# HydrogenSulfate/LFT

Measured on AMD Instinct MI355X. Metric: LF patches/sec (5x5 angRes, 32x32 LR, 4xSR), higher is better.
Workload: dtype bf16; 1 GPU; LFT 5x5 angRes 4xSR inference, batch=4 per GPU, 32x32 LR patches; global_batch=4, parallelism=dp1 (independent shards), streams_per_gpu=1, hip_graph=True, steps_in_flight=2

## Files before the change

lft_amd/csrc/lft_api.hip:

```cpp
#include "../../include/lft_hip.h"
#include "../../include/lft_hip_test.h"
#include <hip/hip_runtime.h>
#include <stdint.h>

#include <cstdarg>
#include <cstdio>
#include <cmath>
#include <map>
#include <mutex>
#include <set>
#include <string>
#include <algorithm>
#include <type_traits>
#include <utility>
#include <vector>

#ifndef LFT_TU
#define LFT_TU 0
#endif

namespace {
#include "lft_kernels_a.cuh"
#include "lft_kernels_b.cuh"
#include "lft_metrics.cuh"
// ... 89 lines not shown

template <auto... Vs, typename V, typename F> int dispatch(V v, F&& f) {
    int rc = 0;
    if (((v == Vs && ((rc = f(std::integral_constant<decltype(Vs), Vs>{})), true)) || ...)) return rc;
    return fail(LFT_ERR_ARG, "internal: no kernel variant for %d", (int)v);
}
template <int V> using int_c = std::integral_constant<int, V>;
template <typename F> int by_prec(int prec, F&& f) {
    if (prec == LFT_PREC_F32) return f(float{});
    if (prec == LFT_PREC_BF16) return f(bf16_t{});
    return f(f16_t{});
}
inline size_t align256(size_t x) { return (x + 255) & ~(size_t)255; }

struct Dims {
    int B, A, V, h, w, hw, s, gp, gt, nchunk;
    long long ntok;
};

int make_dims(int B, int A, int h, int w, int s, int prec, Dims* d) {
    if (prec != LFT_PREC_F32 && prec != LFT_PREC_BF16 && prec != LFT_PREC_F16)
        return fail(LFT_ERR_ARG, "prec must be LFT_PREC_F32, LFT_PREC_BF16 or LFT_PREC_F16, got %d", prec);
    if (B < 1 || A < 1 || h < 1 || w < 1) return fail(LFT_ERR_SHAPE, "B, A, h, w must be positive (B=%d A=%d h=%d w=%d)", B, A, h, w);
    if (s != 2 && s != 4) return fail(LFT_ERR_SHAPE, "scale factor must be 2 or 4, got %d", s);
    if (A * A > 128) return fail(LFT_ERR_UNSUPPORTED, "angRes %d (A*A=%d views > 128) is not implemented in this build", A, A * A);
    if ((long long)B * A * A * h * w > (1LL << 27)) return fail(LFT_ERR_SHAPE, "too many tokens");
    d->B = B; d->A = A; d->V = A * A; d->h = h; d->w = w; d->hw = h * w; d->s = s;
    d->gp = (s + 2) * (s + 2); d->gt = (d->gp + 31) / 32; d->nchunk = 2 * s * s;
    d->ntok = (long long)B * d->V * d->hw;
    return 0;
}

constexpr int kFragsConv = 72, kFragsAng = 64, kFragsSpa1 = 240, kFragsSpa1NoQ = 208, kFragsSpa2 = 176;
inline int frags_up(const Dims& d) { return d.nchunk * (4 + 2 * d.gt); }

struct PackedLayout {
    size_t conv0_w, ln_ang[kLayers], ln_spa[kLayers], ang_pe, petok[kLayers], spa_pe_img;
    size_t w01, s_w01;
    size_t s_conv[3], s_ang[kLayers], s_spa1[kLayers], s_spa2[kLayers], s_up, total;
};

PackedLayout packed_layout(const Dims& d, int prec) {
    const size_t esz = prec == LFT_PREC_F32 ? 4 : 2, fragb = 64 * 8 * esz;
    PackedLayout L;
    size_t o = 0;
    auto take = [&](size_t bytes) { size_t r = o; o = align256(o + bytes); return r; };
    L.conv0_w = take(576 * 4);
    for (int l = 0; l < kLayers; ++l) { L.ln_ang[l] = take(256 * 4); L.ln_spa[l] = take(512 * 4); }
    L.ang_pe = take((size_t)((d.V + 31) / 32) * 2048 * 4);
    for (int l = 0; l < kLayers; ++l) L.petok[l] = take((size_t)((d.hw + 32 * kNwSpa1 - 1) / (32 * kNwSpa1)) * kNwSpa1 * 4096 * esz);
    L.spa_pe_img = take((size_t)d.hw * 64 * esz);
    const bool lp = prec != LFT_PREC_F32;
    L.w01 = take(lp ? 64 * kW01K * 4 : 0);
    L.s_conv[0] = take(kFragsConv * fragb);
    L.s_w01 = take(lp ? kW01Frags * fragb : 0);
    for (int i = 1; i < 3; ++i) L.s_conv[i] = take(kFragsConv * fragb);
    for (int l = 0; l < kLayers; ++l) {
        L.s_ang[l] = take(kFragsAng * fragb);
        L.s_spa1[l] = take(kFragsSpa1 * fragb);
        L.s_spa2[l] = take(kFragsSpa2 * fragb);
    }
    L.s_up = take((size_t)frags_up(d) * fragb);
    L.total = o;
    return L;
}

struct WorkLayout {
    size_t x0, feat, xa, xb, tok, q, k, v, o, g, status, total;
};
WorkLayout work_layout(const Dims& d, int prec) {
    const size_t esz = prec == LFT_PREC_F32 ? 4 : 2;
    WorkLayout W;
    size_t o = 0;
    auto take = [&](size_t bytes) { size_t r = o; o = align256(o + bytes); return r; };
    const size_t n = (size_t)d.ntok;
    W.x0 = take(n * 64 * esz); W.feat = take(n * 64 * esz); W.xa = take(n * 64 * esz); W.xb = take(n * 64 * esz);
    W.tok = take(n * 128 * esz); W.q = take(n * 128 * esz); W.k = take(n * 128 * esz); W.v = take(n * 128 * esz);
    W.o = take(n * 128 * esz);
    W.g = take(n * d.gp * 4);
    W.status = take(256);
    W.total = o;
    return W;
}

template <typename T> size_t lds_conv64(int w) { return WRing<T, kConv64Chunk, kNwConv>::LDS_BYTES + ConvIn<T, kNwConv>::bytes(w) + kNwConv * TileIO<2, T>::BYTES + kConvZeroRow; }
template <typename T> size_t lds_conv64_lr(int w) { return lds_conv64<T>(w) + std::max<size_t>(LrStage<kNwConv>::bytes(w), kConv0WBytes); }
constexpr size_t kLdsParams = 1024;
template <typename T, int CH = kSpaChunk> size_t lds_spa1(int w) {
    return WRing<T, CH, kNwSpa1>::LDS_BYTES + std::max<size_t>(ConvIn<T, kNwSpa1>::bytes(w), (size_t)kNwSpa1 * TileIO<4, T>::BYTES) + kLdsParams + kConvZeroRow;
}
template <typename T> size_t lds_spa2() { return WRing<T, kSpaChunk, kNwSpa2>::LDS_BYTES + kLdsParams + kNwSpa2 * TileIO<4, T>::BYTES; }
template <typename T> size_t lds_up() { return WRing<T, kUpChunk, kNwUp>::LDS_BYTES + kNwUp * TileIO<2, T>::BYTES; }
template <typename T> size_t lds_ang() { return (size_t)kFragsAng * 1024 * FragInfo<T>::PIECES + kLdsParams + 4 * TileIO<2, T>::BYTES; }
constexpr size_t kMaxLds = 160 * 1024;
template <typename K> int allow_lds(K kernel, size_t bytes, const char* name) {
// ... 59 lines not shown
    return dispatch<8, 16>(use8 ? 8 : 16, [&](auto CH) {
        return dispatch<true, false>(lm, [&](auto LM) {
            constexpr bool WQ = !(LM && sizeof(T) == 2);
            const size_t lds = CH == 8 ? l8 : l16;
            if (int rc = allow_lds(k_spa1<T, PE_ONLY, CH, LM, WQ>, lds, "k_spa1")) return rc;
            k_spa1<T, PE_ONLY, CH, LM, WQ><<<nwg, 64 * kNwSpa1, lds, st>>>(in, ws, ln, petok, tok, q, k, v, pe_out, nimg, d.h, d.w, status);
            return 0;
        });
    });
}

template <typename T>
int pack_impl(const float* const* P, void* packed, const Dims& d, int prec, hipStream_t st) {
    const PackedLayout L = packed_layout(d, prec);
    const float kAngScale = 0.35355339059327373f * LFT_LOG2E;
    const float kSpaScale = 0.25f * LFT_LOG2E;
    int rc;
    k_copy_f32<<<3, 256, 0, st>>>(P[0], at<float>(packed, L.conv0_w), 576);
    LFT_LAUNCH_OK("k_copy_f32");
    for (int i = 0; i < 3; ++i) {
        std::vector<PackOp> ops;
        conv_ops(ops, P[1 + i], 64);
        if ((rc = run_pack<T>(ops, at<T>(packed, L.s_conv[i]), kFragsConv, st))) return rc;
    }
    if constexpr (sizeof(T) == 2) {
        k_compose_w01<<<blocks_for(64 * kW01K, 256), 256, 0, st>>>(P[0], P[1], at<float>(packed, L.w01));
        LFT_LAUNCH_OK("k_compose_w01");
        std::vector<PackOp> ops{lin_op(at<float>(packed, L.w01), 0, 64, kW01K, 0, kW01K / 16, 0, 1.0f)};
        if ((rc = run_pack<ConvLrOp>(ops, at<ConvLrOp>(packed, L.s_w01), kW01Frags, st))) return rc;
    }
    k_pe_tables<T><<<blocks_for(std::max<long long>((long long)((d.V + 31) / 32) * 2048, (long long)d.hw * 64), 256), 256, 0, st>>>(
        at<float>(packed, L.ang_pe), at<T>(packed, L.spa_pe_img), d.V, d.h, d.w);
    LFT_LAUNCH_OK("k_pe_tables");
    for (int l = 0; l < kLayers; ++l) {
        const float* const* q = P + 4 + 18 * l;
        float* lnS = at<float>(packed, L.ln_spa[l]);
        float* lnA = at<float>(packed, L.ln_ang[l]);
        const int srcS[4] = {1, 2, 5, 6}, srcA[4] = {10, 11, 14, 15};
        for (int j = 0; j < 4; ++j) {
            k_copy_f32<<<1, 256, 0, st>>>(q[srcS[j]], lnS + 128 * j, 128);
            k_copy_f32<<<1, 256, 0, st>>>(q[srcA[j]], lnA + 64 * j, 64);
        }
        LFT_LAUNCH_OK("k_copy_f32");
        {
            std::vector<PackOp> ops;
            ops.push_back(lin_op(q[12], 0, 64, 64, 0, 4, 1, kAngScale));
            ops.push_back(lin_op(q[12], 64, 64, 64, 0, 4, 1, 1.0f));
            ops.push_back(lin_op(q[12], 128, 64, 64, 0, 4, 1, 1.0f));
            ops.push_back(lin_op(q[13], 0, 64, 64, 0, 4, 1, 1.0f));
            ops.push_back(lin_op(q[16], 0, 128, 64, 0, 4, 1, 1.0f));
            ops.push_back(lin_op(q[17], 0, 64, 128, 0, 8, 1, 1.0f));
            if ((rc = run_pack<T>(ops, at<T>(packed, L.s_ang[l]), kFragsAng, st))) return rc;
        }
        {
            std::vector<PackOp> ops;
            conv_ops(ops, q[0], 128);
            ops.push_back(lin_op(q[3], 256, 128, 128, 0, 8, 1, 1.0f));
            ops.push_back(lin_op(q[3], 128, 128, 128, 0, 8, 1, 1.0f));
            ops.push_back(lin_op(q[3], 0, 128, 128, 0, 8, 1, kSpaScale));
            if ((rc = run_pack<T>(ops, at<T>(packed, L.s_spa1[l]), kFragsSpa1, st))) return rc;
        }
        {
            std::vector<PackOp> ops;
            ops.push_back(lin_op(q[4], 0, 128, 128, 0, 8, (sizeof(T) == 2 && tok_lane_major<T>(d)) ? 1 : 0, 1.0f));
            for (int c = 0; c < 4; ++c) {
                ops.push_back(lin_op(q[7], 64 * c, 64, 128, 0, 8, 1, 1.0f));
                ops.push_back(lin_op(q[8], 0, 128, 256, 64 * c, 4, 1, 1.0f));
            }
            ops.push_back(lin_op(q[9], 0, 64, 128, 0, 8, 1, 1.0f));
            if ((rc = run_pack<T>(ops, at<T>(packed, L.s_spa2[l]), kFragsSpa2, st))) return rc;
        }
        if ((rc = launch_spa1<T, true>((unsigned)((d.hw + 32 * kNwSpa1 - 1) / (32 * kNwSpa1)), at<T>(packed, L.spa_pe_img), at<T>(packed, L.s_spa1[l]), nullptr, nullptr,
                                       nullptr, nullptr, nullptr, nullptr, at<T>(packed, L.petok[l]), 1, d, st, nullptr))) return rc;
        LFT_LAUNCH_OK("k_spa1<pe>");
    }
    {
        std::vector<PackOp> ops;
        for (int c = 0; c < d.nchunk; ++c) {
            ops.push_back(lin_op(P[76], 32 * c, 32, 64, 0, 4, 1, 1.0f));
            PackOp m = lin_op(P[77], 0, d.gp, 0, 32 * c, 2, 1, 1.0f);
            m.kind = 1; m.s = d.s; m.ntiles = d.gt;
            ops.push_back(m);
        }
        if ((rc = run_pack<T>(ops, at<T>(packed, L.s_up), frags_up(d), st))) return rc;
    }
    return 0;
}

void launch_assemble(const float* lr, const float* g, float* out, int B, int A, int h, int w, int s, hipStream_t st, int gld = 0, unsigned* status = nullptr) {
    const dim3 tg((unsigned)((A * w + 7) / 8) * (unsigned)((A * h + 7) / 8) * (unsigned)B);
    if (!gld) gld = (s + 2) * (s + 2);
    if (s == 2) k_assemble_t<2><<<tg, 256, 0, st>>>(lr, g, out, B, A, h, w, gld, status);
    else k_assemble_t<4><<<tg, 256, 0, st>>>(lr, g, out, B, A, h, w, gld, status);
}

template <typename T>
int init_features_x0(const void* packed, const PackedLayout& L, const float* lr, T* x0, T* ta, T* tb, T* feat, const Dims& d, hipStream_t st) {
    const int nimg = d.B * d.V, nwg = nimg * ((d.hw + 32 * kNwConv - 1) / (32 * kNwConv));
    const size_t lds = lds_conv64<T>(d.w);
    int rc;
    if ((rc = allow_lds(k_conv64<T, 0>, lds, "k_conv64"))) return rc;
    if ((rc = allow_lds(k_conv64<T, 1>, lds, "k_conv64"))) return rc;
    k_conv0<T><<<dim3((unsigned)((d.hw + kConv0Tok - 1) / kConv0Tok), (unsigned)nimg), 256, 0, st>>>(lr, at<float>(packed, L.conv0_w), x0, d.B, d.A, d.h, d.w);
// ... 59 lines not shown
}
template <typename T>
int spa_part_a(const void* packed, const PackedLayout& L, int l, const T* in, void* ws, const WorkLayout& W, const Dims& d, hipStream_t st) {
    const int nimg = d.B * d.V, nwg = nimg * ((d.hw + 32 * kNwSpa1 - 1) / (32 * kNwSpa1));
    int rc;
    if ((rc = launch_spa1<T, false>((unsigned)nwg, in, at<T>(packed, L.s_spa1[l]), at<float>(packed, L.ln_spa[l]), at<T>(packed, L.petok[l]),
                                    at<T>(ws, W.tok), at<T>(ws, W.q), at<T>(ws, W.k), at<T>(ws, W.v), nullptr, nimg, d, st, at<unsigned>(ws, W.status)))) return rc;
    LFT_LAUNCH_OK("k_spa1");
    return 0;
}
template <typename F> int with_tail_variant(bool skip, bool tok_lm, bool out_lm, F&& launch) {
    if (out_lm) {
        if (!(skip && tok_lm)) return fail(LFT_ERR_ARG, "internal: lane-major output needs the skip variant and lane-major tokens");
        return launch(std::true_type{}, std::true_type{}, std::true_type{});
    }
    return dispatch<true, false>(skip, [&](auto SK) {
        return dispatch<true, false>(tok_lm, [&](auto LM) { return launch(SK, LM, std::false_type{}); });
    });
}
template <typename T>
int spa_part_b(const void* packed, const PackedLayout& L, int l, const T* skip, T* out, void* ws, const WorkLayout& W,
               const Dims& d, hipStream_t st, bool out_lm = false) {
    const int nimg = d.B * d.V;
    T *tok = at<T>(ws, W.tok), *q = at<T>(ws, W.q), *k = at<T>(ws, W.k), *v = at<T>(ws, W.v), *o = at<T>(ws, W.o);
    const float* ln = at<float>(packed, L.ln_spa[l]);
    const bool lm = tok_lane_major<T>(d);
    int rc;
    if constexpr (sizeof(T) == 2) {
        const unsigned ntile = (unsigned)(nimg * ((d.h + kAttTY - 1) / kAttTY) * ((d.w + kAttTX - 1) / kAttTX));
        if ((rc = with_tail_variant(skip, lm, out_lm, [&](auto SK, auto LM, auto YL) {
                 if (int r = allow_lds(k_spa_b<T, SK, LM, YL>, kSpaBLds, "k_spa_b")) return r;
                 k_spa_b<T, SK, LM, YL><<<ntile, 256, kSpaBLds, st>>>(tok, q, k, v, at<T>(packed, L.s_spa2[l]), ln, skip, out, d.h, d.w,
                                                                      at<unsigned>(ws, W.status), at<T>(packed, L.s_spa1[l]) + (size_t)kFragsSpa1NoQ * 512,
                                                                      at<T>(packed, L.petok[l]));
                 return 0;
             }))) return rc;
        LFT_LAUNCH_OK("k_spa_b");
        return 0;
    } else {
        const unsigned tiles = (unsigned)(((d.w + kWaTX - 1) / kWaTX) * ((d.h + kWaTY - 1) / kWaTY) * nimg);
        if ((rc = allow_lds(k_win_attn_lds<0, true>, kWaLds, "k_win_attn_lds"))) return rc;
        k_win_attn_lds<0, true><<<dim3(tiles, 4), 256, kWaLds, st>>>(reinterpret_cast<const float*>(q), reinterpret_cast<const float*>(k),
                                                                     reinterpret_cast<const float*>(v), reinterpret_cast<float*>(o),
                                                                     nullptr, nullptr, nullptr, nullptr, nullptr, d.h, d.w, 128);
        LFT_LAUNCH_OK("k_spa_attn");
        const unsigned nb = blocks_for(d.ntok, 32 * kNwSpa2);
        if ((rc = with_tail_variant(skip, lm, out_lm, [&](auto SK, auto LM, auto YL) {
                 if (int r = allow_lds(k_spa2<T, SK, LM, YL>, lds_spa2<T>(), "k_spa2")) return r;
                 k_spa2<T, SK, LM, YL><<<nb, 64 * kNwSpa2, lds_spa2<T>(), st>>>(tok, o, at<T>(packed, L.s_spa2[l]), ln, skip, out, d.ntok, at<unsigned>(ws, W.status));
                 return 0;
             }))) return rc;
        LFT_LAUNCH_OK("k_spa2");
        return 0;
    }
}
template <typename T>
int spa_block(const void* packed, const PackedLayout& L, int l, const T* in, const T* skip, T* out, void* ws, const WorkLayout& W,
              const Dims& d, hipStream_t st, bool out_lm = false) {
    int rc;
    if ((rc = spa_part_a<T>(packed, L, l, in, ws, W, d, st))) return rc;
    return spa_part_b<T>(packed, L, l, skip, out, ws, W, d, st, out_lm);
}
template <typename T>
int upsample(const void* packed, const PackedLayout& L, const T* body, const float* lr, float* out, void* ws, const WorkLayout& W,
             const Dims& d, hipStream_t st, bool in_lm = false) {
    float* g = at<float>(ws, W.g);
    const unsigned nb = blocks_for(d.ntok, 32 * kNwUp);
// ... 893 lines not shown
```

lft_amd/csrc/lft_kernels_a.cuh:

```cuda
#pragma once
#include "lft_common.cuh"

struct PackOp {
    const float* src;
    int kind, row0, nrows, ntiles, ld, kmul, kadd, k0, ksteps, kmap, frag0, s;
    float scale;
    int order;
};
__host__ __device__ __forceinline__ int wfrag_index(int OT, int KS, int ot, int ks) {
    const int g = ot >> 2, G = OT - 4 * g < 4 ? OT - 4 * g : 4;
    return 4 * g * KS + ks * G + (ot & 3);
}
__host__ __device__ __forceinline__ void wfrag_coords(int OT, int KS, int lf, int order, int& nt, int& ks) {
    if (!order) { nt = lf / KS; ks = lf % KS; return; }
    const int gl = (OT - 1) >> 2, g = lf / (4 * KS) < gl ? lf / (4 * KS) : gl, G = OT - 4 * g < 4 ? OT - 4 * g : 4, rem = lf - 4 * g * KS;
    ks = rem / G; nt = 4 * g + rem % G;
}
constexpr int LFT_PACK_MAXOPS = 40;
struct PackArgs {
    int nops;
    PackOp op[LFT_PACK_MAXOPS];
};

LFT_DEV float upm_entry(const float* __restrict__ w3, int n, int kk, int s) {
// ... 169 lines not shown
        const char* row = inb ? lds_in + slot * CI::ROW_BYTES : zero_row;
        const int sw = inb ? CI::swz(slot) : 0;
#pragma unroll
        for (int ks = 0; ks < 4; ++ks) {
            Frag<T> b;
            if constexpr (sizeof(T) == 2) {
                b.v = __builtin_bit_cast(typename H16<T>::v8, load_raw16(row + (((2 * ks + hh) ^ sw) * 16)));
            } else {
                b.lo = __builtin_bit_cast(f32x4, load_raw16(row + (((4 * ks + 2 * hh) ^ sw) * 16)));
                b.hi = __builtin_bit_cast(f32x4, load_raw16(row + (((4 * ks + 2 * hh + 1) ^ sw) * 16)));
            }
#pragma unroll
            for (int nt = 0; nt < NT; ++nt) mma(ring.next(), b, acc[nt]);
        }
    }
}

constexpr int kNwConv = 4;
constexpr int kConv64Chunk = 12;

typedef f16_t ConvLrOp;
constexpr int kW01K = 96, kW01Frags = 12;
__host__ __device__ __forceinline__ int conv01_row_channel(int rho) { return (rho & ~12) | ((rho & 4) << 1) | ((rho & 8) >> 1); }
__global__ void k_compose_w01(const float* __restrict__ w0, const float* __restrict__ w1, float* __restrict__ w01) {
    const int idx = blockIdx.x * blockDim.x + threadIdx.x;
    if (idx >= 64 * kW01K) return;
    const int rho = idx / kW01K, k = idx - rho * kW01K;
    float v = 0.0f;
    if (k < 81) {
        const int o = conv01_row_channel(rho), t1 = k / 9, t0 = k - 9 * t1;
        for (int c = 0; c < 64; ++c) v += w1[o * 576 + c * 9 + t1] * w0[c * 9 + t0];
    }
    w01[idx] = v;
}
LFT_DEV const float* lr_view(const float* __restrict__ lr, int im, int A, int h, int w) {
    const int V = A * A, b = im / V, v = im - b * V, a1 = v / A, a2 = v - a1 * A;
    return lr + (size_t)b * (A * h) * (A * w) + (size_t)(a1 * h) * (A * w) + a2 * w;
}
template <int NW> struct LrStage {
    static __host__ __device__ int width(int w) { return w + 4; }
    static __host__ __device__ int max_rows(int w) { return (32 * NW + 2 * w + 1) / w + 6; }
    static __host__ __device__ int bytes(int w) { return (max_rows(w) * width(w) * 4 + 15) & ~15; }
};
constexpr int kConv0WBytes = 9 * 64 * 4;
LFT_DEV void conv0_w_stage(const float* __restrict__ w0, float* wl) {
    float wv[3];
#pragma unroll
    for (int k = 0; k < 3; ++k) wv[k] = w0[min((int)threadIdx.x + 256 * k, 575)];
#pragma unroll
    for (int k = 0; k < 3; ++k) {
        const int i = (int)threadIdx.x + 256 * k, ch = i / 9, t = i - ch * 9;
        if (i < 576) wl[t * 64 + ch] = wv[k];
    }
}
LFT_DEV void conv0_taps_load(const float* __restrict__ img, int ldi, int y, int x, int h, int w, float (&val)[9]) {
#pragma unroll
    for (int t = 0; t < 9; ++t) {
        const int yy = y + t / 3 - 1, xx = x + t % 3 - 1;
        val[t] = img[min(max(yy, 0), h - 1) * ldi + min(max(xx, 0), w - 1)];
    }
}
template <typename T>
LFT_DEV void conv0_token_acc(const float (&tap)[9], const float* wl, int y, int x, int h, int w, int hh, f32x16 (&rr)[2]) {
    float val[9];
#pragma unroll
    for (int t = 0; t < 9; ++t) {
// ... 462 lines not shown
```

lft_amd/csrc/lft_kernels_b.cuh:

```cuda
#pragma once
#include "lft_common.cuh"
#include "lft_kernels_a.cuh"

constexpr int kUpChunk = 8;
constexpr int kSpaChunk = 16;
constexpr int kSpaOcc = 2;
constexpr int kNwSpa1 = 4, kNwSpa2 = 4, kNwUp = 8;
template <typename T, bool PE_ONLY, int CH = kSpaChunk, bool TOKLM = false, bool WITH_Q = true, int NW = kNwSpa1>
__global__ __launch_bounds__(64 * NW, kSpaOcc) void k_spa1(const T* __restrict__ X, const T* __restrict__ ws,
                                              const float* __restrict__ ln, const T* __restrict__ petok,
                                              T* __restrict__ TOK, T* __restrict__ Q, T* __restrict__ K, T* __restrict__ Vv,
                                              T* __restrict__ pe_out, int nimg, int h, int w, unsigned* __restrict__ status) {
    extern __shared__ __attribute__((aligned(16))) char smem[];
    const int lane = threadIdx.x & 63, r = lane & 31, hh = lane >> 5, wave = threadIdx.x >> 6;
    constexpr int TT = 32 * NW;
    const int hw = h * w, tpi = (hw + TT - 1) / TT;
    const int bid = xcd_tile(blockIdx.x, gridDim.x);
    const int im = bid / tpi, p0 = (bid % tpi) * TT;
    const int tl = wave * 32 + r, p = p0 + tl;
    const bool ok = p < hw;
    LFT_STAMP(0);
    typename RawPiece<T>::type pe_raw[16];
    if (!PE_ONLY) load_lane_major_raw<4, T>(petok + (size_t)((p0 >> 5) + wave) * 4096, lane, pe_raw);
    char* lds_in = smem + WRing<T, CH, NW>::LDS_BYTES;
// ... 101 lines not shown
    LFT_STAMP(18);
#pragma unroll
    for (int nt = 0; nt < 4; ++nt) n[nt] = t[nt];
    unsigned bad = 0;
    layernorm_acc<4>(n, lds_ln, lds_ln + 128, hh, bad);
    acc_frags<4, T>(n, f);
    LFT_STAMP(19);
#pragma unroll
    for (int c = 0; c < 4; ++c) {
        f32x16 hid[2];
        zero_acc<2>(hid);
        linear_ring<2, 8, T>(ring, f, hid);
        Frag<T> hf[4];
        acc_frags_relu<2>(hid, hf);
        linear_ring<4, 4, T>(ring, hf, t);
    }
    LFT_STAMP(20);
    acc_frags<4, T>(t, f);
    f32x16 y[2];
    zero_acc<2>(y);
    linear_ring<2, 8, T>(ring, f, y);
    if (SKIP) {
#pragma unroll
        for (int nt = 0; nt < 2; ++nt) y[nt] += sk[nt];
    }
    LFT_STAMP(21);
    if constexpr (YLM) store_tile_lm<2, T>(Y + tb * 64, lane, y);
    else store_tile<2, T>(Y + tb * 64, nvalid, lane, y, scr);
    LFT_STAMP(22);
    publish_status(status, bad);
}

constexpr int kSpaBChunk = 8;
constexpr int kAdTile = kAttHR * kAttHC * 64;
constexpr int kAdPerWave = 2 * kAdTile / 1024 / 4;
static_assert(2 * kAdTile == 4 * kAdPerWave * 1024, "the K and V tiles must split into whole pieces over 4 waves");
constexpr int kSpaBLds = 4 * kAdTile + 2048;
constexpr int kSpaBSlotsA = (2 * kAdTile) / (kSpaBChunk * 1024);
constexpr int kSpaBSlotsB = 2;
constexpr int kSpaBSlots = kSpaBSlotsA + kSpaBSlotsB;
constexpr int kSpaBScratchOfs = 16384;
static_assert(kSpaBScratchOfs + 4 * TileIO<4, bf16_t>::BYTES <= 2 * kAdTile, "scratch must fit buffer B");
static_assert(kSpaBSlotsB * kSpaBChunk * 1024 <= kSpaBScratchOfs, "the ring slots in buffer B must end before the scratch");

template <typename T> LFT_DEV void q_load_async(const T* p0, const T* p1, raw16& a, raw16& b) {
    asm volatile("global_load_dwordx4 %0, %2, off\n\tglobal_load_dwordx4 %1, %3, off" : "=&v"(a), "=&v"(b) : "v"(p0), "v"(p1) : "memory");
}
LFT_DEV void ld16_async(const void* p, raw16& d) { asm volatile("global_load_dwordx4 %0, %1, off" : "=v"(d) : "v"(p) : "memory"); }
template <int OFS> LFT_DEV void ld16_async_ofs(const void* p, raw16& d) {
    static_assert(OFS >= 0 && OFS < 4096, "global_load immediate offset");
    asm volatile("global_load_dwordx4 %0, %1, off offset:%2" : "=v"(d) : "v"(p), "n"(OFS) : "memory");
}
LFT_DEV void ld16_async_x8(const char* p, raw16 (&d)[8]) {
    const char* p2 = p + 4096;
    ld16_async_ofs<0>(p, d[0]); ld16_async_ofs<1024>(p, d[1]); ld16_async_ofs<2048>(p, d[2]); ld16_async_ofs<3072>(p, d[3]);
    ld16_async_ofs<0>(p2, d[4]); ld16_async_ofs<1024>(p2, d[5]); ld16_async_ofs<2048>(p2, d[6]); ld16_async_ofs<3072>(p2, d[7]);
}
template <int N> LFT_DEV void wait_vm_8(raw16 (&r)[8]) {
    asm volatile("s_waitcnt vmcnt(%8)" : "+v"(r[0]), "+v"(r[1]), "+v"(r[2]), "+v"(r[3]), "+v"(r[4]), "+v"(r[5]), "+v"(r[6]), "+v"(r[7]) : "n"(N) : "memory");
    __builtin_amdgcn_sched_barrier(0);
}
template <int N> LFT_DEV void wait_vm_only() {
    asm volatile("s_waitcnt vmcnt(%0)" :: "n"(N) : "memory");
    __builtin_amdgcn_sched_barrier(0);
}
template <int N> LFT_DEV void wait_vm_q(raw16& a, raw16& b) {
    asm volatile("s_waitcnt vmcnt(%2)" : "+v"(a), "+v"(b) : "n"(N) : "memory");
    __builtin_amdgcn_sched_barrier(0);
}

template <typename T> LFT_DEV void q_head_pair(const raw16 (&wr)[8], const Frag<T> (&nf)[8], Frag<T>& q0, Frag<T>& q1) {
    f32x16 q;
#pragma unroll
    for (int i = 0; i < 16; ++i) q[i] = 0.0f;
#pragma unroll
    for (int ks = 0; ks < 8; ++ks) {
        Frag<T> wf;
        wf.v = __builtin_bit_cast(typename H16<T>::v8, wr[ks]);
        mma(wf, nf[ks], q);
    }
    q0 = acc_to_frag(q, 0, T());
    q1 = acc_to_frag(q, 1, T());
}

template <typename T, bool SKIP, bool TOKLM = false, bool YLM = false>
__global__ __launch_bounds__(256, 2) void k_spa_b(const T* __restrict__ TOK, const T* __restrict__ Q, const T* __restrict__ K,
                                                  const T* __restrict__ Vv, const T* __restrict__ ws, const float* __restrict__ ln,
                                                  const T* __restrict__ skip, T* __restrict__ Y, int h, int w, unsigned* __restrict__ status,
                                                  const T* __restrict__ wq, const T* __restrict__ petok) {
    static_assert(sizeof(T) == 2, "k_spa_b is the 16-bit (bf16 / f16) part B; fp32 uses k_win_attn_lds + k_spa2");
    typedef typename H16<T>::v8 V8;
    using Ring = WRingPipe<T, kSpaBChunk, 4, kSpaBSlots, 176>;
    extern __shared__ __attribute__((aligned(16))) char smem[];
    char* const bufA = smem;
    char* const bufB = smem + 2 * kAdTile;
    float* lds_ln = reinterpret_cast<float*>(smem + 4 * kAdTile);
    const int tiles_x = (w + kAttTX - 1) / kAttTX, tiles_y = (h + kAttTY - 1) / kAttTY;
    const int bid = xcd_tile(blockIdx.x, gridDim.x);
    const int tx = bid % tiles_x, ty = (bid / tiles_x) % tiles_y, im = bid / (tiles_x * tiles_y);
    const int lane = threadIdx.x & 63, r = lane & 31, hh = lane >> 5;
    const int wave = __builtin_amdgcn_readfirstlane(threadIdx.x >> 6);
    const int y0 = ty * kAttTY, x0 = tx * kAttTX, bxl = 8 * wave;
    const long long img0 = (long long)im * h * w;
    LFT_STAMP(16);
    const int qpx = 4 * (r >> 4) + (r & 3), qpy = (r >> 2) & 3;
    const int qy = y0 + qpy, qx = x0 + bxl + qpx;
    const long long qtok = img0 + min(qy, h - 1) * w + min(qx, w - 1);
    const T* qptr = TOKLM ? Q + (img0 + (long long)min(qy, h - 1) * w + x0) * 128 + (32 * hh + bxl + qpx) * 8
                               : Q + qtok * 128 + 8 * hh;
    constexpr int kQHead = TOKLM ? 512 : 16, kQPair = 2 * kQHead;
    int dofs[kAdPerWave];
    {
        const int s0 = (wave & 1) * kAdPerWave * 16 + (lane >> 2), piece = lane & 3;
        int row = s0 / kAttHC, col = s0 % kAttHC;
#pragma unroll
        for (int i = 0; i < kAdPerWave; ++i) {
            const int gy = min(max(y0 - 2 + row, 0), h - 1), gx = min(max(x0 - 2 + col, 0), w - 1);
            const int tk = gy * w + gx;
            const int pq = piece ^ att_swz(row, col);
            const int pconst = TOKLM ? ((pq >> 1) * 512 + (pq & 1) * 256) * 2 : pq * 16;
            dofs[i] = (TOKLM ? ((tk & ~31) << 8) + ((tk & 31) << 4) : tk * 256) + pconst;
            col += 16;
            if (col >= kAttHC) { col -= kAttHC; row += 1; }
        }
    }
    constexpr int kDmaPair = TOKLM ? 2048 : 64;
    const char* const dsrc = reinterpret_cast<const char*>((wave < 2 ? K : Vv) + img0 * 128);
    const int ddst = (wave < 2 ? 0 : kAdTile) + (wave & 1) * kAdPerWave * 1024;
    auto stage = [&](int hg, char* buf) {
        LFT_DMA_NOTE("DMA", kNoteKV, hg & 1);
#pragma unroll
        for (int i = 0; i < kAdPerWave; ++i) glds16_asm(dsrc + dofs[i] + hg * kDmaPair, buf + ddst + i * 1024);
    };
    const int g4 = lane >> 4, qi = lane & 15;
    f32x4 bias[2][4];
    int kb[2], vb[2];
    auto setup_tiles = [&]() __attribute__((always_inline)) {
    {
        const int wy0 = max(0, qy - 2), wy1 = min(h, qy + 3), cy0 = y0 - 2;
        const int ya = min(max(wy0 - cy0, 0), 8), yb = min(max(wy1 - cy0, 0), 8);
        const unsigned ymask = ((1u << yb) - 1u) & ~((1u << ya) - 1u);
        const int gy = g4 >> 1, gx4 = 4 * (g4 & 1);
#pragma unroll
        for (int b = 0; b < 2; ++b) {
            const int bqx = x0 + bxl + 4 * b + (lane & 3), cx0 = x0 + bxl + 4 * b - 2;
            const int wx0 = max(0, bqx - 2), wx1 = min(min(h, bqx + 3), w);
            const int xa = min(max(wx0 - cx0, 0), 8), xb = min(max(wx1 - cx0, 0), 8);
            const unsigned xs = (((1u << xb) - 1u) & ~((1u << xa) - 1u)) >> gx4;
#pragma unroll
            for (int t = 0; t < 4; ++t) {
                const unsigned inval = ~(xs & (unsigned)__builtin_amdgcn_sbfe((int)ymask, 2 * t + gy, 1));
#pragma unroll
                for (int e = 0; e < 4; ++e)
                    bias[b][t][e] = __builtin_bit_cast(float, (unsigned)__builtin_amdgcn_sbfe((int)inval, e, 1) & 0xff800000u);
            }
        }
    }
    {
        const int ktok = ((qi >> 3) * kAttHC + bxl + (qi & 7)) * 64, ks0 = (qi >> 3) & 1, ks1 = (qi >> 2) & 1;
        const int vtok = ((g4 >> 1) * kAttHC + bxl + 4 * (g4 & 1) + (qi >> 2)) * 64, vs0 = (g4 >> 1) & 1, vs1 = g4 & 1, vp = qi & 3;
#pragma unroll
        for (int x = 0; x < 2; ++x) {
            kb[x] = ktok + 32 * (x ^ ks1) + 16 * ((g4 >> 1) ^ ks0) + 8 * (g4 & 1);
            vb[x] = kAdTile + vtok + 32 * (x ^ vs1) + 16 * ((vp >> 1) ^ vs0) + 8 * (vp & 1);
        }
    }
    };
    unsigned bad = 0;
    Frag<T> qfr[8];
    raw16 tokr[8];
    raw16 lnv;
    if constexpr (TOKLM) {
        raw16 lnv1, per[8], wqa[8], wqb[8];
        const int ty_ = min(qy, h - 1);
        const int lane_piece = (32 * hh + bxl + qpx) * 8;
        const char* tsrc = reinterpret_cast<const char*>(TOK + (img0 + (long long)ty_ * w + x0) * 128 + lane_piece);
        const char* psrc = reinterpret_cast<const char*>(petok + ((long long)ty_ * w + x0) * 128 + lane_piece);
        const char* wsrc = reinterpret_cast<const char*>(wq) + lane * 16;
        const int pi = min((int)threadIdx.x * 4, 252);
        ld16_async(ln + pi, lnv1);
        ld16_async(ln + 256 + pi, lnv);
        ld16_async_x8(tsrc, tokr);
        ld16_async_x8(psrc, per);
        ld16_async_x8(wsrc, wqa);
        ld16_async_x8(wsrc + 8 * 1024, wqb);
        stage(0, bufA);
        stage(1, bufB);
        wait_vm_8<16 + 2 * kAdPerWave>(tokr);
        wait_vm_8<16 + 2 * kAdPerWave>(per);
        asm volatile("" : "+v"(lnv), "+v"(lnv1));
        params_store(lds_ln, 256, lnv);
        params_store(lds_ln + 256, 256, lnv1);
        wg_barrier_keep_vm();
        f32x16 n[4];
#pragma unroll
        for (int kidx = 0; kidx < 8; ++kidx) {
            const V8 vt = __builtin_bit_cast(V8, tokr[kidx]), vp = __builtin_bit_cast(V8, per[kidx]);
#pragma unroll
            for (int j = 0; j < 8; ++j) n[kidx >> 1][8 * (kidx & 1) + j] = (float)vt[j] + (float)vp[j];
        }
        layernorm_acc<4, true>(n, lds_ln + 256, lds_ln + 256 + 128, hh, bad);
        Frag<T> nf[8];
        acc_frags<4, T>(n, nf);
        wait_vm_8<8 + 2 * kAdPerWave>(wqa);
        q_head_pair<T>(wqa, nf, qfr[0], qfr[1]);
        ld16_async_x8(wsrc + 16 * 1024, wqa);
        wait_vm_8<2 * kAdPerWave + 8>(wqb);
        q_head_pair<T>(wqb, nf, qfr[2], qfr[3]);
        ld16_async_x8(wsrc + 24 * 1024, wqb);
        wait_vm_8<8>(wqa);
        q_head_pair<T>(wqa, nf, qfr[4], qfr[5]);
        wait_vm_8<0>(wqb);
        q_head_pair<T>(wqb, nf, qfr[6], qfr[7]);
#pragma unroll
        for (int hd = 0; hd < 8; ++hd) {
            raw16 f = __builtin_bit_cast(raw16, qfr[hd].v);
            frag_to_blocks(f);
            qfr[hd].v = __builtin_bit_cast(V8, f);
// ... 82 lines not shown
                        V8 ones;
#pragma unroll
                        for (int e = 0; e < 8; ++e) ones[e] = (T)1.0f;
                        osum[b] = mfma16k32(ones, pf, osum[b]);
                    }
                }
                const float inv = osum[b][0] > 0.0f ? fast_rcp(osum[b][0]) : 0.0f;
                V4 oc;
#pragma unroll
                for (int e = 0; e < 4; ++e) oc[e] = (T)(o[e] * inv);
                ob[b] = __builtin_bit_cast(u32x2, oc);
            }
            raw16 fo = raw16{ob[0][0], ob[0][1], ob[1][0], ob[1][1]};
            frag_to_blocks(fo);
            of[2 * hg + hl].v = __builtin_bit_cast(V8, fo);
        }
        LFT_STAMP(19 + 2 * hg);
        LFT_NOTE_ASM_("DONE", kNoteKV, hg & 1);
        wg_barrier_keep_vm();
        if constexpr (!TOKLM) {
            if (hg < 3) q_load_async(qptr + kQPair * (hg + 1), qptr + kQPair * (hg + 1) + kQHead, qa, qb);
        }
        if (hg < 2) stage(hg + 2, buf);
        else if (hg == 2) {
            LFT_NOTE_ASM_("ALIAS_LT", kNoteWRingPipe, kSpaBSlotsA);
#pragma unroll
            for (int c = 0; c < kSpaBSlotsA; ++c) ring.issue(c);
        } else {
#pragma unroll
            for (int c = kSpaBSlotsA; c < kSpaBSlots; ++c) ring.issue(c);
        }
    }
    char* scr = bufB + kSpaBScratchOfs + wave * TileIO<4, T>::BYTES;
    f32x16 t[4], n[4];
    if constexpr (TOKLM) {
#pragma unroll
        for (int kidx = 0; kidx < 8; ++kidx) {
            const V8 v = __builtin_bit_cast(V8, tokr[kidx]);
#pragma unroll
            for (int j = 0; j < 8; ++j) t[kidx >> 1][8 * (kidx & 1) + j] = (float)v[j];
        }
    } else {
        BlkRows rt = rows; rt.img_row_bytes = w * 256; rt.tok_bytes = 256;
        load_tile_map<4, T>(TOK + tok0 * 128, rt, lane, t, scr);
    }
    LFT_STAMP(26);
    __builtin_amdgcn_s_setprio(0);
    ring.start();
    linear_ring_at<0, 4, 8>(ring, of, t);
    LFT_STAMP(27);
#pragma unroll
    for (int nt = 0; nt < 4; ++nt) n[nt] = t[nt];
    layernorm_acc<4, true>(n, lds_ln, lds_ln + 128, hh, bad);
    Frag<T> f[8];
    acc_frags<4, T>(n, f);
    auto ffn_chunk = [&](auto cc) __attribute__((always_inline)) {
        constexpr int C = decltype(cc)::value;
        f32x16 hid[2];
        zero_acc<2>(hid);
        linear_ring_at<32 + 32 * C, 2, 8>(ring, f, hid);
        Frag<T> hf[4];
        acc_frags_relu<2>(hid, hf);
        linear_ring_at<32 + 32 * C + 16, 4, 4>(ring, hf, t);
    };
    ffn_chunk(std::integral_constant<int, 0>());
    ffn_chunk(std::integral_constant<int, 1>());
    ffn_chunk(std::integral_constant<int, 2>());
    ffn_chunk(std::integral_constant<int, 3>());
    LFT_STAMP(28);
    acc_frags<4, T>(t, f);
    f32x16 y[2];
    zero_acc<2>(y);
    linear_ring_at<160, 2, 8>(ring, f, y);
    LFT_STAMP(29);
    BlkRows ry = rows; ry.img_row_bytes = w * 128; ry.tok_bytes = 128;
    if (SKIP) {
        f32x16 sk[2];
        load_tile_map<2, T>(skip + tok0 * 64, ry, lane, sk, scr);
#pragma unroll
        for (int nt = 0; nt < 2; ++nt) y[nt] += sk[nt];
    }
    if constexpr (YLM) {
        if (qy < h) {
            T* dst = Y + (img0 + (long long)qy * w + x0) * 64 + (32 * hh + bxl + qpx) * 8;
#pragma unroll
            for (int kidx = 0; kidx < 4; ++kidx) {
                V8 v;
#pragma unroll
                for (int j = 0; j < 8; ++j) v[j] = (T)y[kidx >> 1][8 * (kidx & 1) + j];
                store_raw16(reinterpret_cast<char*>(dst + kidx * 512), __builtin_bit_cast(raw16, v));
            }
        }
    } else {
        store_tile_map<2, T>(Y + tok0 * 64, ry, lane, y, scr);
    }
    LFT_STAMP(30);
    publish_status(status, bad);
}

template <typename T, int GT, bool XLM = false, int NW = kNwUp>
__global__ __launch_bounds__(64 * NW) void k_up(const T* __restrict__ X, const T* __restrict__ ws, float* __restrict__ G,
                                            long long ntok, int nchunk, int gp) {
    extern __shared__ __attribute__((aligned(16))) char smem[];
    const int lane = threadIdx.x & 63, r = lane & 31, hh = lane >> 5;
    const long long tok_raw = ((long long)blockIdx.x * NW + (threadIdx.x >> 6)) * 32 + r;
    const bool ok = tok_raw < ntok;
// ... 234 lines not shown
```

Baseline: 10260 patches/s.

## Fold output projection into FFN second weight and precompute attention tile geometry

The bf16/f16 spatial part-B kernel now composes the final 128->64 linear with the FFN's second matrix (wl·w2) at pack time. That shrinks the per-token FFN output GEMMs from 128 to 64 columns and removes the trailing projection, so fewer weight fragments stream through the ring. Per-tile DMA offsets, window masks and LDS read bases are precomputed once into a packed geometry table and loaded asynchronously at kernel start, replacing the integer arithmetic done inside the kernel. This adds a pack-time compose kernel and extra global loads, and changes the rounding of the composed weights in low precision.

```diff
diff --git a/lft_amd/csrc/lft_api.hip b/lft_amd/csrc/lft_api.hip
--- a/lft_amd/csrc/lft_api.hip
+++ b/lft_amd/csrc/lft_api.hip
@@ -145,11 +145,14 @@
 }
 
 constexpr int kFragsConv = 72, kFragsAng = 64, kFragsSpa1 = 240, kFragsSpa1NoQ = 208, kFragsSpa2 = 176;
+inline int frags_spa2(int prec) { return prec == LFT_PREC_F32 ? kFragsSpa2 : kSpaBFrags; }
 inline int frags_up(const Dims& d) { return d.nchunk * (4 + 2 * d.gt); }
 
 struct PackedLayout {
     size_t conv0_w, ln_ang[kLayers], ln_spa[kLayers], ang_pe, petok[kLayers], spa_pe_img;
     size_t w01, s_w01;
+    size_t spa_geom;
+    size_t wlw2[kLayers];
     size_t s_conv[3], s_ang[kLayers], s_spa1[kLayers], s_spa2[kLayers], s_up, total;
 };
 
@@ -171,9 +174,12 @@
     for (int l = 0; l < kLayers; ++l) {
         L.s_ang[l] = take(kFragsAng * fragb);
         L.s_spa1[l] = take(kFragsSpa1 * fragb);
-        L.s_spa2[l] = take(kFragsSpa2 * fragb);
+        L.s_spa2[l] = take(frags_spa2(prec) * fragb);
     }
     L.s_up = take((size_t)frags_up(d) * fragb);
+    for (int l = 0; l < kLayers; ++l) L.wlw2[l] = take(lp ? 64 * 256 * 4 : 0);
+    const bool geom = lp && d.hw % (32 * kNwSpa1) == 0 && d.w % 32 == 0;
+    L.spa_geom = take(geom ? (size_t)((d.h + kAttTY - 1) / kAttTY) * ((d.w + kAttTX - 1) / kAttTX) * kSpaBGeomTileBytes : 0);
     L.total = o;
     return L;
 }
@@ -299,6 +305,12 @@
     k_pe_tables<T><<<blocks_for(std::max<long long>((long long)((d.V + 31) / 32) * 2048, (long long)d.hw * 64), 256), 256, 0, st>>>(
         at<float>(packed, L.ang_pe), at<T>(packed, L.spa_pe_img), d.V, d.h, d.w);
     LFT_LAUNCH_OK("k_pe_tables");
+    if constexpr (sizeof(T) == 2) {
+        if (tok_lane_major<T>(d)) {
+            k_spa_b_geom<<<(unsigned)(((d.h + kAttTY - 1) / kAttTY) * ((d.w + kAttTX - 1) / kAttTX)), 256, 0, st>>>(at<unsigned>(packed, L.spa_geom), d.h, d.w);
+            LFT_LAUNCH_OK("k_spa_b_geom");
+        }
+    }
     for (int l = 0; l < kLayers; ++l) {
         const float* const* q = P + 4 + 18 * l;
         float* lnS = at<float>(packed, L.ln_spa[l]);
@@ -330,12 +342,23 @@
         {
             std::vector<PackOp> ops;
             ops.push_back(lin_op(q[4], 0, 128, 128, 0, 8, (sizeof(T) == 2 && tok_lane_major<T>(d)) ? 1 : 0, 1.0f));
-            for (int c = 0; c < 4; ++c) {
-                ops.push_back(lin_op(q[7], 64 * c, 64, 128, 0, 8, 1, 1.0f));
-                ops.push_back(lin_op(q[8], 0, 128, 256, 64 * c, 4, 1, 1.0f));
+            if constexpr (sizeof(T) == 2) {
+                float* wlw2 = at<float>(packed, L.wlw2[l]);
+                k_compose_wlw2<<<blocks_for(64 * 256, 256), 256, 0, st>>>(q[9], q[8], wlw2);
+                LFT_LAUNCH_OK("k_compose_wlw2");
+                ops.push_back(lin_op(q[9], 0, 64, 128, 0, 8, 1, 1.0f));
+                for (int c = 0; c < 4; ++c) {
+                    ops.push_back(lin_op(q[7], 64 * c, 64, 128, 0, 8, 1, 1.0f));
+                    ops.push_back(lin_op(wlw2, 0, 64, 256, 64 * c, 4, 1, 1.0f));
+                }
+            } else {
+                for (int c = 0; c < 4; ++c) {
+                    ops.push_back(lin_op(q[7], 64 * c, 64, 128, 0, 8, 1, 1.0f));
+                    ops.push_back(lin_op(q[8], 0, 128, 256, 64 * c, 4, 1, 1.0f));
+                }
+                ops.push_back(lin_op(q[9], 0, 64, 128, 0, 8, 1, 1.0f));
             }
-            ops.push_back(lin_op(q[9], 0, 64, 128, 0, 8, 1, 1.0f));
-            if ((rc = run_pack<T>(ops, at<T>(packed, L.s_spa2[l]), kFragsSpa2, st))) return rc;
+            if ((rc = run_pack<T>(ops, at<T>(packed, L.s_spa2[l]), frags_spa2(prec), st))) return rc;
         }
         if ((rc = launch_spa1<T, true>((unsigned)((d.hw + 32 * kNwSpa1 - 1) / (32 * kNwSpa1)), at<T>(packed, L.spa_pe_img), at<T>(packed, L.s_spa1[l]), nullptr, nullptr,
                                        nullptr, nullptr, nullptr, nullptr, at<T>(packed, L.petok[l]), 1, d, st, nullptr))) return rc;
@@ -461,7 +484,7 @@
                  if (int r = allow_lds(k_spa_b<T, SK, LM, YL>, kSpaBLds, "k_spa_b")) return r;
                  k_spa_b<T, SK, LM, YL><<<ntile, 256, kSpaBLds, st>>>(tok, q, k, v, at<T>(packed, L.s_spa2[l]), ln, skip, out, d.h, d.w,
                                                                       at<unsigned>(ws, W.status), at<T>(packed, L.s_spa1[l]) + (size_t)kFragsSpa1NoQ * 512,
-                                                                      at<T>(packed, L.petok[l]));
+                                                                      at<T>(packed, L.petok[l]), at<unsigned>(packed, L.spa_geom));
                  return 0;
              }))) return rc;
         LFT_LAUNCH_OK("k_spa_b");
diff --git a/lft_amd/csrc/lft_kernels_a.cuh b/lft_amd/csrc/lft_kernels_a.cuh
--- a/lft_amd/csrc/lft_kernels_a.cuh
+++ b/lft_amd/csrc/lft_kernels_a.cuh
@@ -225,6 +225,14 @@
         for (int c = 0; c < 64; ++c) v += w1[o * 576 + c * 9 + t1] * w0[c * 9 + t0];
     }
     w01[idx] = v;
+}
+__global__ void k_compose_wlw2(const float* __restrict__ wl, const float* __restrict__ w2, float* __restrict__ wlw2) {
+    const int idx = blockIdx.x * blockDim.x + threadIdx.x;
+    if (idx >= 64 * 256) return;
+    const int o = idx >> 8, k = idx & 255;
+    float v = 0.0f;
+    for (int c = 0; c < 128; ++c) v += wl[o * 128 + c] * w2[c * 256 + k];
+    wlw2[idx] = v;
 }
 LFT_DEV const float* lr_view(const float* __restrict__ lr, int im, int A, int h, int w) {
     const int V = A * A, b = im / V, v = im - b * V, a1 = v / A, a2 = v - a1 * A;
diff --git a/lft_amd/csrc/lft_kernels_b.cuh b/lft_amd/csrc/lft_kernels_b.cuh
--- a/lft_amd/csrc/lft_kernels_b.cuh
+++ b/lft_amd/csrc/lft_kernels_b.cuh
@@ -157,6 +157,7 @@
 }
 
 constexpr int kSpaBChunk = 8;
+constexpr int kSpaBFrags = 32 + 16 + 4 * (16 + 8);
 constexpr int kAdTile = kAttHR * kAttHC * 64;
 constexpr int kAdPerWave = 2 * kAdTile / 1024 / 4;
 static_assert(2 * kAdTile == 4 * kAdPerWave * 1024, "the K and V tiles must split into whole pieces over 4 waves");
@@ -189,6 +190,10 @@
     asm volatile("s_waitcnt vmcnt(%0)" :: "n"(N) : "memory");
     __builtin_amdgcn_sched_barrier(0);
 }
+template <int N> LFT_DEV void wait_vm_3(raw16& a, raw16& b, raw16& c) {
+    asm volatile("s_waitcnt vmcnt(%3)" : "+v"(a), "+v"(b), "+v"(c) : "n"(N) : "memory");
+    __builtin_amdgcn_sched_barrier(0);
+}
 template <int N> LFT_DEV void wait_vm_q(raw16& a, raw16& b) {
     asm volatile("s_waitcnt vmcnt(%2)" : "+v"(a), "+v"(b) : "n"(N) : "memory");
     __builtin_amdgcn_sched_barrier(0);
@@ -208,14 +213,74 @@
     q1 = acc_to_frag(q, 1, T());
 }
 
+template <bool TOKLM> LFT_DEV void spa_b_dma_offsets(int wave, int lane, int y0, int x0, int h, int w, int (&dofs)[kAdPerWave]) {
+    const int s0 = (wave & 1) * kAdPerWave * 16 + (lane >> 2), piece = lane & 3;
+    int row = s0 / kAttHC, col = s0 % kAttHC;
+#pragma unroll
+    for (int i = 0; i < kAdPerWave; ++i) {
+        const int gy = min(max(y0 - 2 + row, 0), h - 1), gx = min(max(x0 - 2 + col, 0), w - 1);
+        const int tk = gy * w + gx;
+        const int pq = piece ^ att_swz(row, col);
+        const int pconst = TOKLM ? ((pq >> 1) * 512 + (pq & 1) * 256) * 2 : pq * 16;
+        dofs[i] = (TOKLM ? ((tk & ~31) << 8) + ((tk & 31) << 4) : tk * 256) + pconst;
+        col += 16;
+        if (col >= kAttHC) { col -= kAttHC; row += 1; }
+    }
+}
+LFT_DEV void spa_b_window_masks(int lane, int qy, int y0, int x0, int bxl, int h, int w, unsigned& ymask, unsigned (&xs)[2]) {
+    const int g4 = lane >> 4;
+    const int wy0 = max(0, qy - 2), wy1 = min(h, qy + 3), cy0 = y0 - 2;
+    const int ya = min(max(wy0 - cy0, 0), 8), yb = min(max(wy1 - cy0, 0), 8);
+    ymask = ((1u << yb) - 1u) & ~((1u << ya) - 1u);
+    const int gx4 = 4 * (g4 & 1);
+#pragma unroll
+    for (int b = 0; b < 2; ++b) {
+        const int bqx = x0 + bxl + 4 * b + (lane & 3), cx0 = x0 + bxl + 4 * b - 2;
+        const int wx0 = max(0, bqx - 2), wx1 = min(min(h, bqx + 3), w);
+        const int xa = min(max(wx0 - cx0, 0), 8), xb = min(max(wx1 - cx0, 0), 8);
+        xs[b] = (((1u << xb) - 1u) & ~((1u << xa) - 1u)) >> gx4;
+    }
+}
+LFT_DEV void spa_b_read_bases(int lane, int bxl, int (&kb)[2], int (&vb)[2]) {
+    const int g4 = lane >> 4, qi = lane & 15;
+    const int ktok = ((qi >> 3) * kAttHC + bxl + (qi & 7)) * 64, ks0 = (qi >> 3) & 1, ks1 = (qi >> 2) & 1;
+    const int vtok = ((g4 >> 1) * kAttHC + bxl + 4 * (g4 & 1) + (qi >> 2)) * 64, vs0 = (g4 >> 1) & 1, vs1 = g4 & 1, vp = qi & 3;
+#pragma unroll
+    for (int x = 0; x < 2; ++x) {
+        kb[x] = ktok + 32 * (x ^ ks1) + 16 * ((g4 >> 1) ^ ks0) + 8 * (g4 & 1);
+        vb[x] = kAdTile + vtok + 32 * (x ^ vs1) + 16 * ((vp >> 1) ^ vs0) + 8 * (vp & 1);
+    }
+}
+constexpr int kSpaBGeomPieces = 3, kSpaBGeomTileBytes = 4 * kSpaBGeomPieces * 1024;
+__global__ __launch_bounds__(256) void k_spa_b_geom(unsigned* __restrict__ tab, int h, int w) {
+    const int tiles_x = (w + kAttTX - 1) / kAttTX;
+    const int tile = blockIdx.x, tx = tile % tiles_x, ty = tile / tiles_x;
+    const int lane = threadIdx.x & 63, r = lane & 31, wave = threadIdx.x >> 6;
+    const int y0 = ty * kAttTY, x0 = tx * kAttTX, bxl = 8 * wave;
+    const int qy = y0 + ((r >> 2) & 3);
+    int dofs[kAdPerWave], kb[2], vb[2];
+    unsigned ymask, xs[2];
+    spa_b_dma_offsets<true>(wave, lane, y0, x0, h, w, dofs);
+    spa_b_window_masks(lane, qy, y0, x0, bxl, h, w, ymask, xs);
+    spa_b_read_bases(lane, bxl, kb, vb);
+    unsigned* dst = tab + ((size_t)(tile * 4 + wave) * kSpaBGeomPieces * 64 + lane) * 4;
+#pragma unroll
+    for (int i = 0; i < 8; ++i) dst[(i >> 2) * 256 + (i & 3)] = (unsigned)dofs[i];
+    dst[512] = (unsigned)dofs[8];
+    dst[513] = (unsigned)kb[0] | ((unsigned)kb[1] << 16);
+    dst[514] = (unsigned)vb[0] | ((unsigned)vb[1] << 16);
+    dst[515] = ymask | (xs[0] << 8) | (xs[1] << 16);
+}
+
 template <typename T, bool SKIP, bool TOKLM = false, bool YLM = false>
 __global__ __launch_bounds__(256, 2) void k_spa_b(const T* __restrict__ TOK, const T* __restrict__ Q, const T* __restrict__ K,
                                                   const T* __restrict__ Vv, const T* __restrict__ ws, const float* __restrict__ ln,
                                                   const T* __restrict__ skip, T* __restrict__ Y, int h, int w, unsigned* __restrict__ status,
-                                                  const T* __restrict__ wq, const T* __restrict__ petok) {
+                                                  const T* __restrict__ wq, const T* __restrict__ petok,
+                                                  const unsigned* __restrict__ geom) {
     static_assert(sizeof(T) == 2, "k_spa_b is the 16-bit (bf16 / f16) part B; fp32 uses k_win_attn_lds + k_spa2");
     typedef typename H16<T>::v8 V8;
-    using Ring = WRingPipe<T, kSpaBChunk, 4, kSpaBSlots, 176>;
+    using Ring = WRingPipe<T, kSpaBChunk, 4, kSpaBSlots, kSpaBFrags>;
     extern __shared__ __attribute__((aligned(16))) char smem[];
     char* const bufA = smem;
     char* const bufB = smem + 2 * kAdTile;
@@ -235,20 +300,7 @@
                                : Q + qtok * 128 + 8 * hh;
     constexpr int kQHead = TOKLM ? 512 : 16, kQPair = 2 * kQHead;
     int dofs[kAdPerWave];
-    {
-        const int s0 = (wave & 1) * kAdPerWave * 16 + (lane >> 2), piece = lane & 3;
-        int row = s0 / kAttHC, col = s0 % kAttHC;
-#pragma unroll
-        for (int i = 0; i < kAdPerWave; ++i) {
-            const int gy = min(max(y0 - 2 + row, 0), h - 1), gx = min(max(x0 - 2 + col, 0), w - 1);
-            const int tk = gy * w + gx;
-            const int pq = piece ^ att_swz(row, col);
-            const int pconst = TOKLM ? ((pq >> 1) * 512 + (pq & 1) * 256) * 2 : pq * 16;
-            dofs[i] = (TOKLM ? ((tk & ~31) << 8) + ((tk & 31) << 4) : tk * 256) + pconst;
-            col += 16;
-            if (col >= kAttHC) { col -= kAttHC; row += 1; }
-        }
-    }
+    if constexpr (!TOKLM) spa_b_dma_offsets<false>(wave, lane, y0, x0, h, w, dofs);
     constexpr int kDmaPair = TOKLM ? 2048 : 64;
     const char* const dsrc = reinterpret_cast<const char*>((wave < 2 ? K : Vv) + img0 * 128);
     const int ddst = (wave < 2 ? 0 : kAdTile) + (wave & 1) * kAdPerWave * 1024;
@@ -257,39 +309,30 @@
 #pragma unroll
         for (int i = 0; i < kAdPerWave; ++i) glds16_asm(dsrc + dofs[i] + hg * kDmaPair, buf + ddst + i * 1024);
     };
-    const int g4 = lane >> 4, qi = lane & 15;
+    const int g4 = lane >> 4;
     f32x4 bias[2][4];
     int kb[2], vb[2];
+    raw16 geo2;
     auto setup_tiles = [&]() __attribute__((always_inline)) {
-    {
-        const int wy0 = max(0, qy - 2), wy1 = min(h, qy + 3), cy0 = y0 - 2;
-        const int ya = min(max(wy0 - cy0, 0), 8), yb = min(max(wy1 - cy0, 0), 8);
-        const unsigned ymask = ((1u << yb) - 1u) & ~((1u << ya) - 1u);
-        const int gy = g4 >> 1, gx4 = 4 * (g4 & 1);
-#pragma unroll
-        for (int b = 0; b < 2; ++b) {
-            const int bqx = x0 + bxl + 4 * b + (lane & 3), cx0 = x0 + bxl + 4 * b - 2;
-            const int wx0 = max(0, bqx - 2), wx1 = min(min(h, bqx + 3), w);
-            const int xa = min(max(wx0 - cx0, 0), 8), xb = min(max(wx1 - cx0, 0), 8);
-            const unsigned xs = (((1u << xb) - 1u) & ~((1u << xa) - 1u)) >> gx4;
+        unsigned ymask, xs[2];
+        if constexpr (TOKLM) {
+            ymask = geo2[3] & 0xffu; xs[0] = (geo2[3] >> 8) & 0xffu; xs[1] = geo2[3] >> 16;
+            kb[0] = (int)(geo2[1] & 0xffffu); kb[1] = (int)(geo2[1] >> 16);
+            vb[0] = (int)(geo2[2] & 0xffffu); vb[1] = (int)(geo2[2] >> 16);
+        } else {
+            spa_b_window_masks(lane, qy, y0, x0, bxl, h, w, ymask, xs);
+            spa_b_read_bases(lane, bxl, kb, vb);
+        }
+        const int gy = g4 >> 1;
+#pragma unroll
+        for (int b = 0; b < 2; ++b)
 #pragma unroll
             for (int t = 0; t < 4; ++t) {
-                const unsigned inval = ~(xs & (unsigned)__builtin_amdgcn_sbfe((int)ymask, 2 * t + gy, 1));
+                const unsigned inval = ~(xs[b] & (unsigned)__builtin_amdgcn_sbfe((int)ymask, 2 * t + gy, 1));
 #pragma unroll
                 for (int e = 0; e < 4; ++e)
                     bias[b][t][e] = __builtin_bit_cast(float, (unsigned)__builtin_amdgcn_sbfe((int)inval, e, 1) & 0xff800000u);
             }
-        }
-    }
-    {
-        const int ktok = ((qi >> 3) * kAttHC + bxl + (qi & 7)) * 64, ks0 = (qi >> 3) & 1, ks1 = (qi >> 2) & 1;
-        const int vtok = ((g4 >> 1) * kAttHC + bxl + 4 * (g4 & 1) + (qi >> 2)) * 64, vs0 = (g4 >> 1) & 1, vs1 = g4 & 1, vp = qi & 3;
-#pragma unroll
-        for (int x = 0; x < 2; ++x) {
-            kb[x] = ktok + 32 * (x ^ ks1) + 16 * ((g4 >> 1) ^ ks0) + 8 * (g4 & 1);
-            vb[x] = kAdTile + vtok + 32 * (x ^ vs1) + 16 * ((vp >> 1) ^ vs0) + 8 * (vp & 1);
-        }
-    }
     };
     unsigned bad = 0;
     Frag<T> qfr[8];
@@ -303,12 +346,20 @@
         const char* psrc = reinterpret_cast<const char*>(petok + ((long long)ty_ * w + x0) * 128 + lane_piece);
         const char* wsrc = reinterpret_cast<const char*>(wq) + lane * 16;
         const int pi = min((int)threadIdx.x * 4, 252);
+        raw16 geo0, geo1;
+        const char* gsrc = reinterpret_cast<const char*>(geom) + (size_t)(bid % (tiles_x * tiles_y)) * kSpaBGeomTileBytes
+                           + wave * (kSpaBGeomPieces * 1024) + lane * 16;
+        ld16_async_ofs<0>(gsrc, geo0); ld16_async_ofs<1024>(gsrc, geo1); ld16_async_ofs<2048>(gsrc, geo2);
         ld16_async(ln + pi, lnv1);
         ld16_async(ln + 256 + pi, lnv);
         ld16_async_x8(tsrc, tokr);
         ld16_async_x8(psrc, per);
         ld16_async_x8(wsrc, wqa);
         ld16_async_x8(wsrc + 8 * 1024, wqb);
+        wait_vm_3<2 + 32>(geo0, geo1, geo2);
+#pragma unroll
+        for (int i = 0; i < 4; ++i) { dofs[i] = (int)geo0[i]; dofs[4 + i] = (int)geo1[i]; }
+        dofs[8] = (int)geo2[0];
         stage(0, bufA);
         stage(1, bufB);
         wait_vm_8<16 + 2 * kAdPerWave>(tokr);
@@ -457,7 +508,7 @@
         }
     }
     char* scr = bufB + kSpaBScratchOfs + wave * TileIO<4, T>::BYTES;
-    f32x16 t[4], n[4];
+    f32x16 t[4];
     if constexpr (TOKLM) {
 #pragma unroll
         for (int kidx = 0; kidx < 8; ++kidx) {
@@ -474,29 +525,27 @@
     ring.start();
     linear_ring_at<0, 4, 8>(ring, of, t);
     LFT_STAMP(27);
-#pragma unroll
-    for (int nt = 0; nt < 4; ++nt) n[nt] = t[nt];
-    layernorm_acc<4, true>(n, lds_ln, lds_ln + 128, hh, bad);
     Frag<T> f[8];
-    acc_frags<4, T>(n, f);
+    acc_frags<4, T>(t, f);
+    f32x16 y[2];
+    zero_acc<2>(y);
+    linear_ring_at<32, 2, 8>(ring, f, y);
+    layernorm_acc<4, true>(t, lds_ln, lds_ln + 128, hh, bad);
+    acc_frags<4, T>(t, f);
     auto ffn_chunk = [&](auto cc) __attribute__((always_inline)) {
         constexpr int C = decltype(cc)::value;
         f32x16 hid[2];
         zero_acc<2>(hid);
-        linear_ring_at<32 + 32 * C, 2, 8>(ring, f, hid);
+        linear_ring_at<48 + 24 * C, 2, 8>(ring, f, hid);
         Frag<T> hf[4];
         acc_frags_relu<2>(hid, hf);
-        linear_ring_at<32 + 32 * C + 16, 4, 4>(ring, hf, t);
+        linear_ring_at<48 + 24 * C + 16, 2, 4>(ring, hf, y);
     };
     ffn_chunk(std::integral_constant<int, 0>());
     ffn_chunk(std::integral_constant<int, 1>());
     ffn_chunk(std::integral_constant<int, 2>());
     ffn_chunk(std::integral_constant<int, 3>());
     LFT_STAMP(28);
-    acc_frags<4, T>(t, f);
-    f32x16 y[2];
-    zero_acc<2>(y);
-    linear_ring_at<160, 2, 8>(ring, f, y);
     LFT_STAMP(29);
     BlkRows ry = rows; ry.img_row_bytes = w * 128; ry.tok_bytes = 128;
     if (SKIP) {
```

After: 10540 patches/s, median of 6. +2.7%, better.
